# koide3/fast_gicp

Measured on AMD Instinct MI355X. Metric: registrations/sec (100-iter reuse) + final fitness_score; achieved HBM GB/s, higher is better.
Workload: dtype f64

## Files before the change

### fast_gicp_amd/csrc/host_runtime.inc.hpp

```cpp


constexpr int MAX_COST_BLOCKS = MAX_PARTIAL_ROWS;

struct DevBuf {
  void* p = nullptr;
  size_t cap = 0;
  hipError_t ensure(size_t bytes) {
    if (bytes <= cap) return hipSuccess;
    if (p) { hipError_t e = hipFree(p); p = nullptr; cap = 0; if (e != hipSuccess) return e; }
    size_t want = bytes + bytes / 4 + 256;
    hipError_t e = hipMalloc(&p, want);
    if (e == hipSuccess) cap = want;
    return e;
  }
  void release() { if (p) (void)hipFree(p); p = nullptr; cap = 0; }
  template <typename T> T* as() const { return reinterpret_cast<T*>(p); }
};

inline const char* fvh_env(const char* name) { return getenv(name); }
inline long long fvh_env_ll(const char* name, long long dflt) { const char* v = fvh_env(name); return v ? atoll(v) : dflt; }
inline unsigned long long fvh_env_ull(const char* name, unsigned long long dflt) { const char* v = fvh_env(name); return v ? strtoull(v, nullptr, 10) : dflt; }
constexpr int COHERENT_MIN_POINTS = 32768;
struct ProcessParams { int slot_max_split, contended_slot_pct, xcd_local, small_grid_layout; };
inline const ProcessParams& process_params() {
  static const ProcessParams p = [] {
    ProcessParams q;
    q.slot_max_split = (int)std::max(1LL, fvh_env_ll("FVH_SLOT_MAX_SPLIT", 4));
    q.contended_slot_pct = (int)std::min(100LL, std::max(10LL, fvh_env_ll("FVH_CONTENDED_SLOT_PCT", 100)));
    q.xcd_local = fvh_env_ll("FVH_XCD_LOCAL", 1) != 0 ? 1 : 0;
    q.small_grid_layout = fvh_env_ll("FVH_SMALL_GRID_LAYOUT", 2) == 0 ? 0 : 2;
    return q;
  }();
  return p;
}
inline const fvh_engine_params& env_engine_defaults() {
  static const fvh_engine_params d = [] {
    fvh_engine_params p;
    std::memset(&p, 0, sizeof(p));
    p.struct_size = (int)sizeof(fvh_engine_params);
    p.sort_mode = (int)fvh_env_ll("FVH_SORT_MODE", 2);
    p.sort_items = (int)fvh_env_ll("FVH_SORT_ITEMS", 0);
    { const int b = (int)fvh_env_ll("FVH_SORT_FUSED_BITS", 10); p.sort_fused_bits = (b == 9 || b == 10) ? b : 0; }
    p.sort_two_pass_max = (int)fvh_env_ll("FVH_SORT_TWO_PASS_MAX", 262144);
    p.sort_coop_watchdog_ticks = 2'000'000ull;
    p.knn_nearest_first_max_points = (int)fvh_env_ll("FVH_KNN_NEAREST_FIRST_MAX_POINTS", 65536);
    { const int b = (int)fvh_env_ll("FVH_KNN_BLOCK", 64); p.knn_block = (b == 256 || b == 128) ? b : 64; }
    p.coherent_min_points = (int)fvh_env_ll("FVH_COHERENT_MIN_POINTS", COHERENT_MIN_POINTS);
    p.bitmap_min_points = (int)fvh_env_ll("FVH_BITMAP_MIN_POINTS", 300000);
    p.bitmap_max_bytes = std::min(fvh_env_ull("FVH_BITMAP_MAX_BYTES", 32ull << 20), 16ull << 30);
    p.persistent = (int)fvh_env_ll("FVH_PERSISTENT", 1);
    p.persist_watchdog_ticks = 5'000'000ull;
    p.peer_watchdog_ticks = fvh_env_ull("FVH_PEER_WATCHDOG_TICKS", 200'000'000ull);
    p.lm_everywhere = (int)fvh_env_ll("FVH_LM_EVERYWHERE", 1);
    { const char* v = fvh_env("FVH_COST_PRIO"); p.cost_prio = v ? (atoi(v) != 0 ? 1 : 0) : -1; }
    p.cost_split = (int)fvh_env_ll("FVH_COST_SPLIT", 1);
    p.cost_group_max = (int)std::min<long long>(std::max(1LL, fvh_env_ll("FVH_COST_GROUP_MAX", COST_CH)), COST_CH);
    { const long long b = fvh_env_ll("FVH_COST_MAX_BLOCKS", MAX_PARTIAL_ROWS); p.cost_max_blocks = (int)(b < 1 ? 1 : (b > MAX_PARTIAL_ROWS ? MAX_PARTIAL_ROWS : b)); }
    p.cost_target_items = fvh_env_ll("FVH_COST_TARGET_ITEMS", 256LL * 256 * 2);
    p.zerocopy_result = (int)fvh_env_ll("FVH_ZEROCOPY_RESULT", 1);
    { const char* v = fvh_env("FVH_HOST_WAIT"); p.host_wait_block = (v && std::string(v) == "block") ? 1 : 0; }
    p.result_query_spins = fvh_env_ull("FVH_RESULT_QUERY_SPINS", 1024ull);
    p.side_stream = fvh_env_ll("FVH_SIDE_STREAM", 1) != 0 ? 1 : 0;
    p.pinned_upload_max = fvh_env_ull("FVH_PINNED_UPLOAD_MAX", 8ull << 20);
    p.zerocopy_upload_max = fvh_env_ull("FVH_ZEROCOPY_UPLOAD_MAX", 1ull << 20);
    p.avg_fused = fvh_env_ll("FVH_AVG_FUSED", 1) != 0 ? 1 : 0;
    p.nn1_seed = fvh_env_ll("FVH_NN1_SEED", 1) != 0 ? 1 : 0;
    return p;
  }();
  return d;
}
inline const char* check_engine_params(const fvh_engine_params& p) {
  if (p.struct_size != (int)sizeof(fvh_engine_params)) return "engine params: struct_size does not match this library's fvh_engine_params (start from fvh_default_engine_params / fvh_*_get_engine_params)";
  if (p.sort_mode < 0 || p.sort_mode > 3) return "engine params: sort_mode must be 0..3";
  if (p.sort_fused_bits != 0 && p.sort_fused_bits != 9 && p.sort_fused_bits != 10) return "engine params: sort_fused_bits must be 0, 9 or 10";
  if (p.knn_block != 64 && p.knn_block != 128 && p.knn_block != 256) return "engine params: knn_block must be 64, 128 or 256";
  if (p.cost_group_max < 1 || p.cost_group_max > COST_CH) return "engine params: cost_group_max must be 1..4";
  if (p.cost_max_blocks < 1 || p.cost_max_blocks > MAX_PARTIAL_ROWS) return "engine params: cost_max_blocks must be 1..1024";
  if (p.cost_target_items < 1) return "engine params: cost_target_items must be positive";
  if (p.lm_everywhere < 0 || p.lm_everywhere > 2 || p.cost_prio < -1 || p.cost_prio > 1) return "engine params: lm_everywhere must be 0..2, cost_prio -1..1";
  if (p.bitmap_max_bytes > (16ull << 30)) return "engine params: bitmap_max_bytes beyond 16 GiB (the LM kernel indexes its words with 32 bits)";
  if (p.sort_items < 0 || p.sort_items > SORT_ITEMS_MAX || (p.sort_items & 63)) return "engine params: sort_items must be 0 or a multiple of 64 up to 1024";
  return nullptr;
}
// ... 118 lines not shown
  Grant acquire(int dev, int cap, int want) {
    std::lock_guard<std::mutex> lk(mu);
    dev &= 15;
    const auto now = std::chrono::steady_clock::now();
    active[dev]++;
    if (active[dev] > 1) last_contention[dev] = now;
    else if (recent[dev] > 1 && now - last_contention[dev] > std::chrono::milliseconds(QUIET_RESET_MS)) { recent[dev] = 1; calm[dev] = 0; }
    recent[dev] = std::max(recent[dev], active[dev]);
    const int max_split = process_params().slot_max_split;
    const int contended_pct = process_params().contended_slot_pct;
    const bool contended = recent[dev] > 1;
    const int pool = contended ? cap * contended_pct / 100 : cap;
    const int share = std::max(1, pool / std::max(1, std::min(recent[dev], max_split)));
    Grant g;
    g.n = std::min(std::min(want, share), std::max(0, cap - reserved[dev]));
    if (g.n < std::min(want, 32)) {
      active[dev]--;
      calm[dev] = 0;
      last_contention[dev] = now;
      return Grant{};
    }
    reserved[dev] += g.n;
    return g;
  }
  void snapshot(int dev, int* res, int* act, int* rec) {
    std::lock_guard<std::mutex> lk(mu);
    dev &= 15;
    *res = reserved[dev]; *act = active[dev]; *rec = recent[dev];
  }
  void release(int dev, const Grant& g) {
    std::lock_guard<std::mutex> lk(mu);
    dev &= 15;
    reserved[dev] -= g.n;
    active[dev]--;
    if (recent[dev] > active[dev] + 1) {
      if (++calm[dev] >= DECAY_AFTER) { recent[dev]--; calm[dev] = 0; }
    } else {
      calm[dev] = 0;
    }
  }
};
SlotPool g_slots;
constexpr int XCD_LOCAL_MAX_STRIKES = 3;
std::atomic<int> g_xcd_local_strikes{0};
inline bool xcd_local_wanted() {
  return process_params().xcd_local && g_xcd_local_strikes.load() < XCD_LOCAL_MAX_STRIKES;
}
struct GridPlan { int nb = 0; int ng = 0; int local = 0; };
inline int small_grid_layout() {
  return process_params().small_grid_layout;
}
inline int default_groups(int nb) {
  if (nb > SINGLE_LEVEL_MAX_BLOCKS) return TICKET_GROUPS;
  return (small_grid_layout() == 2 && nb >= 2 * TICKET_GROUPS) ? TICKET_GROUPS : 1;
}
```

### fast_gicp_amd/csrc/kernels_cost.hpp

```cpp
#pragma once
#include <cstddef>
#include <type_traits>

#include "dev_math.hpp"
#include "kernels_peer.hpp"
#include "kernels_voxelmap.hpp"

#pragma clang fp contract(on)

namespace fvh {

constexpr int NSUM = 28;
constexpr int PART_STRIDE = 32;
constexpr int MAX_PARTIAL_ROWS = 1024;

enum CostMode { MODE_VGICP = 0, MODE_NDT_P2D = 1, MODE_NDT_D2D = 2 };
enum Phase { PH_LINEARIZE = 0, PH_TRIAL = 1, PH_DONE = 2, PH_FIND_ONLY = 3, PH_EVAL_DERIV = 4, PH_EVAL_ERROR = 5,
             PH_TRIAL_FINAL = 6 };

struct LmState {
  PoseD x0;
  PoseD xi;
  PoseD x_lin;
  double H[36], b[6], d[6];
// ... 140 lines not shown
  if (__builtin_amdgcn_ballot_w64(rot_eps > 0 && trans_eps > 0) != 0ull) {
    bool ok = true;
#pragma unroll
    for (int i = 0; i < 9; i++) ok &= (fabs(delta.r[i] - ((i % 4 == 0) ? 1.0 : 0.0)) < rot_eps);
#pragma unroll
    for (int i = 0; i < 3; i++) ok &= (fabs(delta.t[i]) < trans_eps);
    return ok;
  }
  double rmax = 0, tmax = 0;
#pragma unroll
  for (int i = 0; i < 9; i++) rmax = fmax(rmax, fabs(delta.r[i] - ((i % 4 == 0) ? 1.0 : 0.0)));
#pragma unroll
  for (int i = 0; i < 3; i++) tmax = fmax(tmax, fabs(delta.t[i]));
  const double qr = rmax / rot_eps, qt = tmax / trans_eps;
  return (qr < qt ? qt : qr) < 1;
}

__device__ __host__ inline void unpack_sums(const double* s, double* H, double* b) {
  for (int i = 0; i < 6; i++) b[i] = s[1 + i];
  const double* rr = s + 7;
  const double* rt = s + 13;
  const double* tt = s + 22;
  const int sym[3][3] = {{0, 1, 2}, {1, 3, 4}, {2, 4, 5}};
  for (int i = 0; i < 3; i++)
    for (int j = 0; j < 3; j++) {
      H[i * 6 + j] = rr[sym[i][j]];
      H[i * 6 + 3 + j] = rt[i * 3 + j];
      H[(3 + j) * 6 + i] = rt[i * 3 + j];
      H[(3 + i) * 6 + 3 + j] = tt[sym[i][j]];
    }
}
__device__ __host__ constexpr int sums_index_of_H(int i, int j) {
  const int a = i < 3 ? i : i - 3, c = j < 3 ? j : j - 3;
  const int lo = a < c ? a : c, hi = a < c ? c : a;
  const int sym = lo * 3 - (lo * (lo - 1)) / 2 + (hi - lo);
  return (i < 3 && j < 3) ? 7 + sym : (i >= 3 && j >= 3) ? 22 + sym : (i < 3) ? 13 + i * 3 + (j - 3) : 13 + j * 3 + (i - 3);
}

#ifdef FVH_LM_STEP_NOINLINE
#define FVH_LM_STEP_ATTR __noinline__
#else
#define FVH_LM_STEP_ATTR __forceinline__
#endif
#define FVH_UNI(c) (__builtin_amdgcn_ballot_w64(c) != 0ull)
#ifdef FVH_COST_TIMING
__device__ unsigned long long g_lmtime[16][8];
__device__ unsigned g_lmcall;
#endif
#if defined(FVH_COST_TIMING) && defined(FVH_LM_STAGES)
#define FVH_LM_T(k) do { asm volatile("s_waitcnt vmcnt(0) lgkmcnt(0)" ::: "memory"); if (lane == 0 && lm_call < 16) g_lmtime[lm_call][k] = __builtin_readcyclecounter(); } while (0)
#else
#define FVH_LM_T(k) do { } while (0)
#endif
template <bool GN = false>
__device__ FVH_LM_STEP_ATTR void dev_lm_step_wave(LmState* st, const double* sums, const int lane, double* trace = nullptr) {
  const bool in36 = lane < 36, in12 = lane < 12, in6 = lane < 6;
  double* x0p = reinterpret_cast<double*>(&st->x0);
  double* xip = reinterpret_cast<double*>(&st->xi);
  double* xlp = reinterpret_cast<double*>(&st->x_lin);
#if defined(FVH_COST_TIMING) && defined(FVH_LM_STAGES)
  const unsigned lm_call = __builtin_amdgcn_readfirstlane(g_lmcall);
  if (lane == 0) g_lmcall = lm_call + 1;
#endif
  FVH_LM_T(0);
  const int phase0 = __builtin_amdgcn_readfirstlane(st->phase);
  int phase = phase0;
  double lambda = st->lambda, nu = st->nu, y0 = st->y0;
  int outer_iter = __builtin_amdgcn_readfirstlane(st->outer_iter), inner_iter = __builtin_amdgcn_readfirstlane(st->inner_iter);
  int converged = __builtin_amdgcn_readfirstlane(st->converged), lm_failed = __builtin_amdgcn_readfirstlane(st->lm_failed);
  int num_linearize = __builtin_amdgcn_readfirstlane(st->num_linearize), num_error_evals = __builtin_amdgcn_readfirstlane(st->num_error_evals);
  int nr_iterations = __builtin_amdgcn_readfirstlane(st->nr_iterations), corr_cur = __builtin_amdgcn_readfirstlane(st->corr_cur);
  const int max_iterations = __builtin_amdgcn_readfirstlane(st->max_iterations), lm_max_iterations = __builtin_amdgcn_readfirstlane(st->lm_max_iterations);
  constexpr bool gauss_newton = GN;
  const double rot_eps = st->rotation_epsilon, trans_eps = st->transformation_epsilon, lambda_factor = st->lm_init_lambda_factor;
  double dprev[6], bprev[6];
#pragma unroll
  for (int j = 0; j < 6; j++) { dprev[j] = st->d[j]; bprev[j] = st->b[j]; }
  const int delta_conv_prev = __builtin_amdgcn_readfirstlane(st->delta_converged);

  const double s0 = sums[0], s28 = sums[28];
  if (lane == 0 && sums[30] > 0.0) st->halo_exceeded = 1;

  bool accepted = false, consume = false, done = false;
  if (phase0 == PH_LINEARIZE) {
    consume = true;
  } else {
    const double yi = phase0 == PH_TRIAL_FINAL ? s0 : s28;
    num_error_evals++;
    double denom = 0;
#pragma unroll
    for (int j = 0; j < 6; j++) denom += dprev[j] * (lambda * dprev[j] - bprev[j]);
    double rho;
    if (FVH_UNI(fabs(denom) > 1e-290)) rho = (y0 - yi) * fast_rcp(denom); else rho = (y0 - yi) / denom;
    if (trace) {
      double dn = 0;
#pragma unroll
      for (int j = 0; j < 6; j++) dn += dprev[j] * dprev[j];
      if (lane == 0) {
        double* row = trace + 6 * (size_t)(num_error_evals - 1);
        row[0] = (double)inner_iter; row[1] = y0; row[2] = yi; row[3] = rho; row[4] = lambda; row[5] = sqrt(dn);
      }
    }
    const bool conv = delta_conv_prev != 0;
    if (FVH_UNI(rho < 0)) {
      if (conv) {
        converged = 1; outer_iter++; phase = PH_DONE; done = true;
      } else {
        lambda = nu * lambda;
        nu = 2 * nu;
        inner_iter++;
        if (inner_iter >= lm_max_iterations) { lm_failed = 1; phase = PH_DONE; done = true; }
      }
    } else {
      accepted = true;
      { const double u = 2 * rho - 1; lambda = lambda * fmax(1.0 / 3.0, 1 - u * u * u); }
      converged = conv ? 1 : 0;
      outer_iter++;
      if (converged || outer_iter >= max_iterations) {
        phase = PH_DONE; done = true;
      } else {
        corr_cur ^= 1;
        consume = true;
      }
    }
  }
  FVH_LM_T(1);
  double Hl[21], bv[6];
  if (!done) {
    if (consume) {
      y0 = s0;
#pragma unroll
      for (int i = 0; i < 6; i++) {
        bv[i] = sums[1 + i];
#pragma unroll
        for (int j = 0; j <= i; j++) Hl[i * (i + 1) / 2 + j] = sums[sums_index_of_H(i, j)];
      }
      num_linearize++;
      nr_iterations = outer_iter;
      if (FVH_UNI(lambda < 0.0)) {
        double mx = 0;
#pragma unroll
        for (int i = 0; i < 6; i++) mx = fmax(mx, fabs(Hl[i * (i + 1) / 2 + i]));
        lambda = lambda_factor * mx;
      }
      nu = 2.0;
      inner_iter = 0;
      if (phase0 == PH_LINEARIZE && !gauss_newton) {
        if (lm_max_iterations <= 0) { lm_failed = 1; phase = PH_DONE; done = true; } else phase = PH_TRIAL;
      }
    } else {
#pragma unroll
      for (int i = 0; i < 6; i++) {
        bv[i] = bprev[i];
#pragma unroll
        for (int j = 0; j <= i; j++) Hl[i * (i + 1) / 2 + j] = st->H[i * 6 + j];
      }
    }
  }
  if (lane == 0) { st->lambda = lambda; st->nu = nu; st->y0 = y0; }
  FVH_LM_T(2);
  PoseD delta;
  double d[6];
  bool gn_step = false;
  int delta_conv = delta_conv_prev;
  if (!done) {
    double L[15], D[6], Dinv[6];
    const double lam_solve = gauss_newton ? 0.0 : lambda;
#pragma unroll
    for (int j = 0; j < 6; j++) {
      double dj = Hl[j * (j + 1) / 2 + j] + lam_solve;
#pragma unroll
      for (int k = 0; k < j; k++) dj -= L[j * (j - 1) / 2 + k] * L[j * (j - 1) / 2 + k] * D[k];
      D[j] = dj;
      const double r = fast_rcp(dj);
      const bool pivot_ok = fabs(dj) > 2.2250738585072014e-308;
      Dinv[j] = pivot_ok ? r : 0.0;
      const double scale = pivot_ok ? r : 1.0;
#pragma unroll
      for (int i = j + 1; i < 6; i++) {
        double sacc = Hl[i * (i + 1) / 2 + j];
#pragma unroll
        for (int k = 0; k < j; k++) sacc -= L[i * (i - 1) / 2 + k] * L[j * (j - 1) / 2 + k] * D[k];
        L[i * (i - 1) / 2 + j] = sacc * scale;
      }
    }
    double y[6];
#pragma unroll
    for (int i = 0; i < 6; i++) {
      double sacc = -bv[i];
#pragma unroll
      for (int k = 0; k < i; k++) sacc -= L[i * (i - 1) / 2 + k] * y[k];
      y[i] = sacc;
    }
#pragma unroll
    for (int i = 0; i < 6; i++) y[i] *= Dinv[i];
#pragma unroll
    for (int i = 5; i >= 0; i--) {
      double sacc = y[i];
#pragma unroll
      for (int k = i + 1; k < 6; k++) sacc -= L[k * (k - 1) / 2 + i] * d[k];
      d[i] = sacc;
    }
    FVH_LM_T(3);
    dev_se3_exp(d, delta);
    FVH_LM_T(4);
    delta_conv = FVH_UNI(dev_is_converged(rot_eps, trans_eps, delta)) ? 1 : 0;
    if (gauss_newton) {
      gn_step = true;
      converged = delta_conv;
      outer_iter++;
      phase = (converged || outer_iter >= max_iterations) ? PH_DONE : PH_LINEARIZE;
    } else {
      phase = (delta_conv || outer_iter + 1 >= max_iterations) ? PH_TRIAL_FINAL : PH_TRIAL;
    }
  }
  FVH_LM_T(5);
  double x0r[12], xir[12];
  {
    const double* src = accepted ? xip : x0p;
#pragma unroll
    for (int k = 0; k < 12; k++) x0r[k] = src[k];
  }
  if (accepted && in36) st->final_H[lane] = st->H[lane];
  if (consume) {
    const int li = lane / 6, lj = lane - li * 6;
    const int a = li < 3 ? li : li - 3, c = lj < 3 ? lj : lj - 3;
    const int lo = a < c ? a : c, hi = a < c ? c : a;
    const int sym = lo * 3 - (lo * (lo - 1)) / 2 + (hi - lo);
    int hidx;
    if (li < 3 && lj < 3) hidx = 7 + sym;
    else if (li >= 3 && lj >= 3) hidx = 22 + sym;
    else if (li < 3) hidx = 13 + li * 3 + (lj - 3);
    else hidx = 13 + lj * 3 + (li - 3);
    if (in36) st->H[lane] = sums[hidx];
    if (in6) st->b[lane] = sums[1 + lane];
    if (gn_step && in36) st->final_H[lane] = sums[hidx];
  }
  if (!done) {
#pragma unroll
    for (int i = 0; i < 3; i++) {
#pragma unroll
      for (int j = 0; j < 3; j++) xir[i * 3 + j] = delta.r[i * 3 + 0] * x0r[0 * 3 + j] + delta.r[i * 3 + 1] * x0r[1 * 3 + j] + delta.r[i * 3 + 2] * x0r[2 * 3 + j];
      xir[9 + i] = delta.r[i * 3 + 0] * x0r[9] + delta.r[i * 3 + 1] * x0r[10] + delta.r[i * 3 + 2] * x0r[11] + delta.t[i];
    }
  }
  if (lane == 0) {
    if (accepted) {
#pragma unroll
      for (int k = 0; k < 12; k++) x0p[k] = x0r[k];
    }
    if (consume) {
#pragma unroll
      for (int k = 0; k < 12; k++) xlp[k] = (gn_step && phase != PH_DONE) ? xir[k] : x0r[k];
    }
    if (gn_step) {
#pragma unroll
      for (int k = 0; k < 12; k++) x0p[k] = xir[k];
    }
    if (!done) {
#pragma unroll
      for (int k = 0; k < 12; k++) xip[k] = xir[k];
#pragma unroll
      for (int j = 0; j < 6; j++) st->d[j] = d[j];
    }
    st->phase = phase;
    st->outer_iter = outer_iter; st->inner_iter = inner_iter; st->converged = converged; st->lm_failed = lm_failed;
    st->num_linearize = num_linearize; st->num_error_evals = num_error_evals; st->nr_iterations = nr_iterations; st->corr_cur = corr_cur;
    st->delta_converged = delta_conv;
  }
  FVH_LM_T(6);
}

__global__ void lm_init_kernel(LmState* st, PoseD guess, double rot_eps, double trans_eps, double lambda_factor, int max_iter, int lm_max_iter, unsigned* ticket, int optimizer = 0) {
  if (blockIdx.x == 0 && threadIdx.x <= 8) ticket[threadIdx.x] = 0;
  if (threadIdx.x != 0 || blockIdx.x != 0) return;
  st->x0 = guess; st->xi = guess;
  st->rotation_epsilon = rot_eps; st->transformation_epsilon = trans_eps; st->lm_init_lambda_factor = lambda_factor;
  st->max_iterations = max_iter; st->lm_max_iterations = lm_max_iter; st->optimizer = optimizer; st->pad_ = 0;
  st->lambda = -1.0; st->nu = 2.0; st->y0 = 0.0;
  st->phase = max_iter > 0 ? PH_LINEARIZE : PH_DONE;
  st->corr_cur = 0; st->x_lin = guess; st->delta_converged = 0; st->halo_exceeded = 0;
  st->outer_iter = 0; st->inner_iter = 0; st->converged = 0; st->lm_failed = 0; st->num_linearize = 0; st->num_error_evals = 0; st->nr_iterations = 0;
  for (int i = 0; i < 36; i++) st->final_H[i] = (i % 7 == 0) ? 1.0 : 0.0;
}
template <bool GN = false>
__global__ __launch_bounds__(64) void lm_update_kernel(LmState* st) {
  __shared__ LmState s;
  constexpr int WORDS = sizeof(LmState) / 8 - 1;
  unsigned long long* g = reinterpret_cast<unsigned long long*>(st);
  unsigned long long* l = reinterpret_cast<unsigned long long*>(&s);
  for (int i = threadIdx.x; i < WORDS; i += 64) l[i] = g[i];
  __syncthreads();
  if (s.phase == PH_DONE) return;
  dev_lm_step_wave<GN>(&s, s.sums, threadIdx.x);
  __syncthreads();
  for (int i = threadIdx.x; i < WORDS; i += 64) g[i] = l[i];
}

template <typename Real>
struct ItemAcc {
  Sym3<Real> S;
  Vec3<Real> g;
  Real err;
};
template <typename Real>
__device__ __forceinline__ void hit_term(ItemAcc<Real>& it, const Vec3<Real>& q, const Vec3<Real>& mu, const Sym3<Real>& A, Real w, bool deriv) {
  const Vec3<Real> e = {mu.x - q.x, mu.y - q.y, mu.z - q.z};
  Real det;
  const Sym3<Real> C = adjugate(A, det);
  const Real s = fast_div(w, det);
  const Vec3<Real> Ce = mul(C, e);
  it.err += s * (e.x * Ce.x + e.y * Ce.y + e.z * Ce.z);
  if (!deriv) return;
  it.g.x += s * Ce.x; it.g.y += s * Ce.y; it.g.z += s * Ce.z;
  it.S.xx += s * C.xx; it.S.xy += s * C.xy; it.S.xz += s * C.xz; it.S.yy += s * C.yy; it.S.yz += s * C.yz; it.S.zz += s * C.zz;
}
template <typename Real>
__device__ __forceinline__ Real record_weight(const float4& q3) { return (Real)__hiloint2double(__float_as_int(q3.w), __float_as_int(q3.z)); }
template <typename Real>
__device__ __forceinline__ Real record_weight(const float2&) { return (Real)1; }
template <typename Real>
__device__ __forceinline__ void item_sums(double* v, const ItemAcc<Real>& it, const Vec3<Real>& q) {
  v[0] = (double)it.err;
  const Vec3<Real> bq = cross(it.g, q);
  v[1] = (double)bq.x; v[2] = (double)bq.y; v[3] = (double)bq.z;
  v[4] = -(double)it.g.x; v[5] = -(double)it.g.y; v[6] = -(double)it.g.z;
  const Sym3<Real>& S = it.S;
  const Vec3<Real> c0 = {S.xx, S.xy, S.xz}, c1 = {S.xy, S.yy, S.yz}, c2 = {S.xz, S.yz, S.zz};
  const Vec3<Real> p0 = cross(q, c0), p1 = cross(q, c1), p2 = cross(q, c2);
  const Vec3<Real> r0 = {p0.x, p1.x, p2.x}, r1 = {p0.y, p1.y, p2.y}, r2 = {p0.z, p1.z, p2.z};
  const Vec3<Real> h0 = cross(q, r0), h1 = cross(q, r1), h2 = cross(q, r2);
  v[7] = (double)h0.x; v[8] = (double)h0.y; v[9] = (double)h0.z; v[10] = (double)h1.y; v[11] = (double)h1.z; v[12] = (double)h2.z;
  v[13] = (double)r0.x; v[14] = (double)r0.y; v[15] = (double)r0.z;
  v[16] = (double)r1.x; v[17] = (double)r1.y; v[18] = (double)r1.z;
  v[19] = (double)r2.x; v[20] = (double)r2.y; v[21] = (double)r2.z;
  v[22] = (double)S.xx; v[23] = (double)S.xy; v[24] = (double)S.xz; v[25] = (double)S.yy; v[26] = (double)S.yz; v[27] = (double)S.zz;
}

__device__ __forceinline__ int probe_continue(const unsigned long long* __restrict__ keys, unsigned mask, unsigned long long key, unsigned slot) {
  for (unsigned it = 0; it < mask; it++) {
    slot = (slot + 1) & mask;
    const unsigned long long k = keys[slot];
    if (k == key) return (int)slot;
    if (k == FVH_EMPTY_KEY) return -1;
  }
  return -1;
}
// ... 84 lines not shown
#ifdef FVH_ASM_MARKS
#define FVH_MT(trip, k) asm volatile("; FVH_MARK " #k)
#define FVH_MARK(k) asm volatile("; FVH_MARK " #k)
#else
#define FVH_MT(trip, k) do { } while (0)
#endif
#endif
#ifndef FVH_MARK
#define FVH_MARK(k) do { } while (0)
#endif

#ifndef FVH_COST_WG_PER_CU
#define FVH_COST_WG_PER_CU 3
#endif
#define FVH_COST_BOUNDS __launch_bounds__(256, FVH_COST_WG_PER_CU)
template <typename Real> using LdsPose = const Pose<Real> __attribute__((address_space(3)))*;
typedef const int __attribute__((address_space(3)))* LdsInt;
template <typename Real>
__device__ __forceinline__ Pose<Real> lds_pose(LdsPose<Real> p, int which) {
  Pose<Real> o;
#pragma unroll
  for (int k = 0; k < 9; k++) o.r[k] = p[which].r[k];
#pragma unroll
  for (int k = 0; k < 3; k++) o.t[k] = p[which].t[k];
  return o;
}

constexpr size_t GANG_TICKET_WORDS = 16;
constexpr size_t GANG_BCAST_DOUBLES = (size_t)PERSIST_REPLICAS * BCAST_PAIRS * 2;
constexpr size_t GANG_RESULT_WORDS = (sizeof(LmState) / 8 + 1 + 7) & ~(size_t)7;
constexpr int MAX_GANGS = 64;
struct GangParams {
  int nb_h;
  const PoseD* guesses;
};

template <typename Real, int MODE, bool PERSIST, int CH, bool GN, bool GANG>
__device__ __forceinline__ void cost_body(const CostParams& P, const unsigned gang_lb, const unsigned gang_nb, const unsigned gang, const PoseD* gang_guesses) {
  static_assert(CH == 1 || CH == COST_CH, "one or COST_CH lookups per item");
  auto lin_arg = [&]() -> PoseD { if constexpr (GANG) return gang_guesses[gang]; else return P.lin; };
  auto partials = [&]() -> double* { if constexpr (GANG) return P.partials + (size_t)gang * PARTIALS_DOUBLES; else return P.partials; };
  auto ticket = [&]() -> unsigned* { if constexpr (GANG) return P.ticket + (size_t)gang * GANG_TICKET_WORDS; else return P.ticket; };
  auto bcast_base = [&]() -> double* { if constexpr (GANG) return P.bcast + (size_t)gang * GANG_BCAST_DOUBLES; else return P.bcast; };
  auto corr_base = [&]() -> int* { if constexpr (GANG) return P.corr + (size_t)gang * 2 * P.corr_stride; else return P.corr; };
  auto result_host = [&]() -> unsigned long long* { if constexpr (GANG) return P.result_host ? P.result_host + (size_t)gang * GANG_RESULT_WORDS : nullptr; else return P.result_host; };
#ifdef FVH_COST_TIMING
  __shared__ unsigned long long stamp[12];
  if (threadIdx.x == 0) { stamp[0] = wall_clock64(); atomicMin(&g_cost_timing[0], stamp[0]); }
#endif
  __shared__ double red[4][PART_STRIDE];
  __shared__ double fin[8][PART_STRIDE];
  __shared__ int s_last;
  __shared__ LmState s_st;
  static_assert(sizeof(LmState) % 8 == 0, "LmState is copied as 64-bit words");
  constexpr int ST_WORDS = sizeof(LmState) / 8 - 1;
  static_assert(ST_WORDS <= 256, "one state word per thread after the barrier");
  LmState* st = GANG ? P.st + gang : P.st;
  unsigned long long* st_words = reinterpret_cast<unsigned long long*>(st);
  const unsigned lb = GANG ? gang_lb : blockIdx.x, nb = GANG ? gang_nb : gridDim.x;
  unsigned gen = 0;
  int phase, corr_sel;
  PoseD lin_d, ev_d;
  if (P.host_phase >= 0) {
    phase = P.host_phase;
    lin_d = P.lin;
    ev_d = P.ev;
    corr_sel = P.host_corr_sel;
  } else if (P.init) {
    phase = PH_LINEARIZE;
    lin_d = lin_arg();
    ev_d = lin_arg();
    corr_sel = 0;
  } else {
    phase = st->phase;
    if (phase == PH_DONE) return;
    lin_d = st->x_lin;
    ev_d = (phase == PH_LINEARIZE) ? st->x0 : st->xi;
    corr_sel = st->corr_cur;
  }
  __shared__ Pose<Real> s_pose[2];
  if (threadIdx.x == 0) { s_pose[0] = pose_cast<Real>(lin_d); s_pose[1] = pose_cast<Real>(ev_d); }
  __shared__ int s_grid[8];
  __shared__ int s_region[8];
  constexpr int OFFP_LDS = 64;
  __shared__ int s_offp[OFFP_LDS];
  if (threadIdx.x >= 64 && threadIdx.x < 64 + OFFP_LDS) s_offp[threadIdx.x - 64] = ((int)threadIdx.x - 64 < P.n_off) ? P.offsets_packed[threadIdx.x - 64] : 0;
  if (threadIdx.x < 8) {
    const int t = threadIdx.x;
    int gv = 0, rv = 0;
    if (P.bitmap && P.grid) gv = t < 3 ? P.grid->b0[t] : (t < 6 ? P.grid->nb[t - 3] : (t == 6 ? P.grid->enabled : 0));
    if (P.region) rv = t < 3 ? P.region->inner_lo[t] : (t < 6 ? P.region->inner_hi[t - 3] : 0);
    s_grid[t] = gv; s_region[t] = rv;
  }
  __syncthreads();
  const int n_src_launch = P.d_n_src ? *P.d_n_src : P.n_src;
  constexpr int STICKY_T = PERSIST ? 256 : 1;
  __shared__ float4 s_src[3][STICKY_T];
  constexpr int ELEM_ITS = 2;
  __shared__ int s_elem[PERSIST ? ELEM_ITS : 1][STICKY_T];
  __shared__ int s_ids[2][CH][STICKY_T];
  __shared__ int s_ofp[CH][STICKY_T];
  bool a_primed = false;
  for (;;) {
  if (PERSIST) FVH_PT_MIN(gen, 0);
  const bool fused = (P.host_phase < 0) && (phase == PH_TRIAL);
  constexpr bool EXT_OK = !PERSIST && MODE == MODE_VGICP;
// ... 406 lines not shown
      double s = 0.0;
#pragma unroll
      for (int c = 0; c < 8; c++) s += fin[c][v];
      red[0][v] = s;
    }
  };
  auto init_state = [&]() {
    s_st.x0 = lin_arg(); s_st.xi = lin_arg(); s_st.x_lin = lin_arg();
    s_st.rotation_epsilon = P.rotation_epsilon; s_st.transformation_epsilon = P.transformation_epsilon; s_st.lm_init_lambda_factor = P.lm_init_lambda_factor;
    s_st.max_iterations = P.max_iterations; s_st.lm_max_iterations = P.lm_max_iterations; s_st.optimizer = P.optimizer; s_st.pad_ = 0;
    s_st.lambda = -1.0; s_st.nu = 2.0; s_st.y0 = 0.0;
    s_st.phase = PH_LINEARIZE; s_st.corr_cur = 0; s_st.delta_converged = 0; s_st.halo_exceeded = 0;
    s_st.outer_iter = 0; s_st.inner_iter = 0; s_st.converged = 0; s_st.lm_failed = 0; s_st.num_linearize = 0; s_st.num_error_evals = 0; s_st.nr_iterations = 0;
    for (int i = 0; i < 36; i++) s_st.final_H[i] = (i % 7 == 0) ? 1.0 : 0.0;
  };

  if constexpr (!PERSIST) {
    if (tid == 0) s_last = (atomicAdd(&ticket()[grp], 1u) == gsize - 1);
    __syncthreads();
    if (!s_last) return;
    FVH_STAMP(3);
    reduce_group_rows((size_t)MAX_PARTIAL_ROWS + grp);
    if (tid == 0) s_last = (atomicAdd(&ticket()[TICKET_GROUPS], 1u) == ngroups - 1);
    __syncthreads();
    if (!s_last) return;
    FVH_STAMP(4);

    reduce_final((size_t)MAX_PARTIAL_ROWS);
    if (tid <= TICKET_GROUPS) ticket()[tid] = 0;
    if (MODE == MODE_VGICP && P.peer.n > 1) {
      __syncthreads();
      if (!peer_exchange_sums(P.peer, red[0], P.peer.xbase, P.peer_watchdog_ticks, tid, 256, &s_last)) {
        if (tid == 0) __hip_atomic_store(&st->aborted, 2u, __ATOMIC_RELAXED, __HIP_MEMORY_SCOPE_AGENT);
        return;
      }
    }
    for (int i = tid; i < ST_WORDS; i += 256) reinterpret_cast<unsigned long long*>(&s_st)[i] = st_words[i];
    int vm_nv = 0, vm_dr = 0, vm_nv2 = 0;
    if (tid == 0) {
      vm_nv = P.vm_counters[0];
      vm_nv2 = P.vm_counters2 ? P.vm_counters2[0] : 0;
      vm_dr = P.vm_counters[1] + (P.vm_counters2 ? P.vm_counters2[1] : 0);
    }
    __syncthreads();
    FVH_STAMP(5);
    if (tid == 0) {
      for (int v = 0; v < PART_STRIDE; v++) s_st.sums[v] = red[0][v];
      s_st.vm_num_voxels = vm_nv;
      s_st.vm_num_voxels2 = vm_nv2;
      s_st.vm_dropped = vm_dr;
      if (P.host_phase < 0 && P.init) init_state();
    }
    __syncthreads();
    if (P.host_phase < 0 && !P.defer_lm && tid < 64) dev_lm_step_wave<GN>(&s_st, red[0], tid, P.lm_trace);
    FVH_STAMP(6);
    __syncthreads();
    for (int i = tid; i < ST_WORDS; i += 256) st_words[i] = reinterpret_cast<const unsigned long long*>(&s_st)[i];
#ifdef FVH_COST_TIMING
    asm volatile("s_waitcnt vmcnt(0)" ::: "memory");
    if (tid == 0) {
      stamp[7] = wall_clock64();
      for (int i = 1; i <= 7; i++) g_cost_timing[i] = stamp[i];
      g_cost_timing[8] = nb;
      g_cost_timing[9] = stamp[0];
    }
#endif
    return;
  } else {
    const unsigned trip = gen;
    unsigned long long ltag = P.launch_tag;
    asm volatile("" : "+s"(ltag));
    auto want_tag_of = [&]() { unsigned long long t = ltag * 4096ull + trip + 1; asm volatile("" : "+s"(t)); return (double)t; };
    auto abort_tag_of = [&]() { unsigned long long t = ltag * 4096ull; asm volatile("" : "+s"(t)); return -(double)t; };
    __shared__ double bc[BCAST_PAIRS];
    __shared__ unsigned s_abort;
    pair_t* wrows = reinterpret_cast<pair_t*>(partials() + WG_ROWS_OFFSET);
    pair_t* trows = reinterpret_cast<pair_t*>(partials() + TAGGED_ROWS_OFFSET) + (size_t)(trip & 1u) * (TICKET_GROUPS + 1) * PART_STRIDE;
    pair_t* bcast = reinterpret_cast<pair_t*>(bcast_base());
    const bool local = P.xcd_local != 0;
    const unsigned reps = NG == 1 ? (unsigned)PERSIST_REPLICAS : (unsigned)(PERSIST_REPLICAS / TICKET_GROUPS);
    static_assert(PERSIST_REPLICAS % (2 * TICKET_GROUPS) == 0, "an even number of broadcast copies per group");
    pair_t* my_bcast = bcast + (size_t)(NG == 1 ? 0u : grp * reps) * BCAST_PAIRS;
    auto poison = [&](int first, int stride) {
      pair_t pv;
      pv.x = 0.0; pv.y = abort_tag_of();
      for (int idx = first; idx < PERSIST_REPLICAS * BCAST_PAIRS; idx += stride) store_pair_agent(bcast + idx, pv);
    };
    const double my_rot = local ? (double)((__builtin_amdgcn_readfirstlane(xcc_id()) - blockIdx.x) & 7u) : 0.0;
    if (tid < PART_STRIDE) {
      pair_t pv;
      pv.x = (red[0][tid] + red[1][tid]) + (red[2][tid] + red[3][tid]);
      if (tid == PART_STRIDE - 1) pv.x = my_rot;
      pv.y = want_tag_of();
      if (local) store_pair_xcd(wrows + (size_t)lb * PART_STRIDE + tid, pv); else store_pair_agent(wrows + (size_t)lb * PART_STRIDE + tid, pv);
    }
    FVH_PT_MAX(trip, 2);
    const bool collector = lb < NG;
    const bool multi_gpu = MODE == MODE_VGICP && P.peer.n > 1;
    const bool everywhere = P.lm_everywhere != 0 && !multi_gpu;
    const bool adds_rows = collector;
    if (collector || everywhere) {
      if (tid == 0) { s_last = 1; s_abort = 0u; }
      __syncthreads();
      if (adds_rows) {
        const int v = tid & 31, chunk = tid >> 5;
        const double want = want_tag_of();
        double s = 0.0;
        for (unsigned j0 = chunk; j0 < gsize; j0 += 8 * 8) {
          const pair_t* src[8];
          double t[8];
          unsigned pend = 0;
#pragma unroll
          for (int u = 0; u < 8; u++) {
            const unsigned j = j0 + 8 * u;
            const bool in = j < gsize;
            src[u] = wrows + (size_t)(grp + (in ? j : j0) * NG) * PART_STRIDE + v;
            t[u] = 0.0;
            pend |= in ? (1u << u) : 0u;
          }
          const unsigned long long t0 = wall_clock64();
          for (;;) {
            pair_t pv[8];
            load_pairs8_agent(pv, src);
#pragma unroll
            for (int u = 0; u < 8; u++)
              if (((pend >> u) & 1u) && pv[u].y == want) { t[u] = pv[u].x; pend &= ~(1u << u); }
            if (!pend) break;
            if (wall_clock64() - t0 > P.watchdog_ticks) { s_last = 0; break; }
            __builtin_amdgcn_s_sleep(1);
          }
          if (v == PART_STRIDE - 1) {
#pragma unroll
            for (int u = 0; u < 8; u++) t[u] = (((j0 + 8 * u) < gsize) && t[u] != my_rot) ? 1.0 : 0.0;
          }
#pragma unroll
          for (int u = 0; u < 8; u++) s += t[u];
        }
        fin[chunk][v] = s;
      }
      if (adds_rows) __syncthreads();
      if (!s_last) {
        poison(tid, 256);
        if (tid == 0) __hip_atomic_store(&st->aborted, 1u, __ATOMIC_RELAXED, __HIP_MEMORY_SCOPE_AGENT);
        return;
      }
      if (adds_rows && tid < PART_STRIDE) {
        double s = 0.0;
#pragma unroll
        for (int c = 0; c < 8; c++) s += fin[c][tid];
        if (tid == PART_STRIDE - 1) s = (s == 0.0) ? my_rot : -1.0;
        if (NG > 1) {
          pair_t pv;
          pv.x = s; pv.y = want_tag_of();
          store_pair_agent(trows + (size_t)grp * PART_STRIDE + tid, pv);
        }
        red[1][tid] = s;
      }
      FVH_PT_MAX(trip, 5);
      if (tid < 64) {
        const int lane = tid;
        double val = 0.0;
        bool ok = true;
        if (NG == 1) {
          if (lane < PART_STRIDE) val = red[1][lane];
        } else if (!multi_gpu || lb == 0) {
          const pair_t* src[8];
          double t[8];
          unsigned pend = 0;
#pragma unroll
          for (int g = 0; g < 8; g++) {
            const bool in = (unsigned)g < NG;
            src[g] = trows + (size_t)(in ? g : 0) * PART_STRIDE + (lane & 31);
            t[g] = 0.0;
            pend |= in ? (1u << g) : 0u;
          }
          if (lane >= PART_STRIDE) pend = 0;
          const double want = want_tag_of();
          const unsigned long long t0 = wall_clock64();
          while (__builtin_amdgcn_ballot_w64(pend != 0u) != 0ull) {
            pair_t pv[8];
            load_pairs8_agent(pv, src);
#pragma unroll
            for (int g = 0; g < 8; g++)
              if (((pend >> g) & 1u) && pv[g].y == want) { t[g] = pv[g].x; pend &= ~(1u << g); }
            if (__builtin_amdgcn_readfirstlane((int)(wall_clock64() - t0 > P.watchdog_ticks))) { ok = false; break; }
          }
          if (lane == PART_STRIDE - 1) {
#pragma unroll
            for (int g = 0; g < 8; g++) t[g] = ((unsigned)g < NG && t[g] != my_rot) ? 1.0 : 0.0;
          }
#pragma unroll
          for (int g = 0; g < 8; g++) val += t[g];
        } else {
          const pair_t* src = trows + (size_t)GLOBAL_ROW * PART_STRIDE + (lane & 31);
          const double want = want_tag_of();
          const unsigned long long t0 = wall_clock64();
          bool pend = lane < PART_STRIDE;
          while (__builtin_amdgcn_ballot_w64(pend) != 0ull) {
            const pair_t pv = load_pair_agent(src);
            if (pend && pv.y == want) { val = pv.x; pend = false; }
            if (__builtin_amdgcn_readfirstlane((int)(wall_clock64() - t0 > P.watchdog_ticks))) { ok = false; break; }
          }
        }
        FVH_PT_MAX(trip, 6);
        if (lane == PART_STRIDE - 1) {
          const bool placement_ok = !local || (NG == 1 ? val == my_rot : val == 0.0);
          if (ok && !placement_ok) s_abort = 3u;
          val = 0.0;
        }
        if (lane < PART_STRIDE) red[0][lane] = val;
        if (!ok && lane == 0) s_abort = 1u;
      }
      if (multi_gpu && lb == 0) {
        __syncthreads();
        if constexpr (MODE == MODE_VGICP) {
          if (!s_abort && !peer_exchange_sums(P.peer, red[0], P.peer.xbase + trip, P.peer_watchdog_ticks, tid, 256, &s_last)) {
            if (tid == 0) s_abort = 2u;
          }
        }
        __syncthreads();
        if (!s_abort && NG > 1 && tid < PART_STRIDE) {
          pair_t pv;
          pv.x = red[0][tid]; pv.y = want_tag_of();
          store_pair_agent(trows + (size_t)GLOBAL_ROW * PART_STRIDE + tid, pv);
        }
      }
      if (tid < 64) {
        const int lane = tid;
        if (__builtin_amdgcn_ballot_w64(s_abort != 0u) == 0ull) {
          FVH_PT_MAX(trip, 7);
          if (trip == 0 && lane == 0) {
            init_state();
            s_st.vm_num_voxels = P.vm_counters[0];
            s_st.vm_num_voxels2 = P.vm_counters2 ? P.vm_counters2[0] : 0;
            s_st.vm_dropped = P.vm_counters[1] + (P.vm_counters2 ? P.vm_counters2[1] : 0);
          }
          if (lane < PART_STRIDE) s_st.sums[lane] = red[0][lane];
          FVH_PT_MAX(trip, 8);
          FVH_MARK(20);
#ifdef FVH_COST_TIMING
          const unsigned long long lm_c0 = __builtin_readcyclecounter();
#endif
          dev_lm_step_wave<GN>(&s_st, red[0], lane, lb == 0 ? P.lm_trace : nullptr);
#ifdef FVH_COST_TIMING
          if (threadIdx.x == 0 && trip < 16 && lb == 0) g_ptime[trip][0][11] = __builtin_readcyclecounter() - lm_c0;
#endif
          FVH_MARK(21);
          FVH_PT_MAX(trip, 9);
          const int ph = __builtin_amdgcn_readfirstlane(s_st.phase);
          double v = 0.0;
          const int d = lane & 31;
          if (d < BCAST_VALUES) {
            const double* xl = reinterpret_cast<const double*>(&s_st.x_lin);
            const double* pe = reinterpret_cast<const double*>(ph == PH_LINEARIZE ? &s_st.x0 : &s_st.xi);
            if (d == 0) v = (double)ph;
            else if (d == 1) v = (double)s_st.corr_cur;
            else if (d < 14) v = xl[d - 2];
            else v = pe[d - 14];
            if (lane < 32) bc[d] = v;
            pair_t pv;
            pv.x = v; pv.y = want_tag_of();
            pair_t* dst = my_bcast + lane;
            static_assert(BCAST_PAIRS == 32, "two copies per store instruction");
            if (everywhere) {
            } else if (local) {
              for (unsigned r = 0; r < reps; r += 2) store_pair_xcd(dst + (size_t)r * BCAST_PAIRS, pv);
            } else {
              for (unsigned r = 0; r < reps; r += 2) store_pair_agent(dst + (size_t)r * BCAST_PAIRS, pv);
            }
          }
          FVH_PT_MAX(trip, 3);
        }
      }
      __syncthreads();
      if (s_abort) {
        poison(tid, 256);
        if (tid == 0) __hip_atomic_store(&st->aborted, s_abort, __ATOMIC_RELAXED, __HIP_MEMORY_SCOPE_AGENT);
        return;
      }
      if (lb == 0 && s_st.phase == PH_DONE) {
        for (int i = tid; i < ST_WORDS; i += 256) st_words[i] = reinterpret_cast<const unsigned long long*>(&s_st)[i];
        if (result_host()) {
          for (int i = tid; i < ST_WORDS; i += 256)
            __hip_atomic_store(&result_host()[i], reinterpret_cast<const unsigned long long*>(&s_st)[i], __ATOMIC_RELAXED, __HIP_MEMORY_SCOPE_SYSTEM);
          asm volatile("s_waitcnt vmcnt(0)" ::: "memory");
          __syncthreads();
          if (tid == 0) __hip_atomic_store(&result_host()[ST_WORDS + 1], P.launch_tag, __ATOMIC_RELEASE, __HIP_MEMORY_SCOPE_SYSTEM);
        }
      }
    } else {
      if (tid < 64) {
        const pair_t* rep = my_bcast + (size_t)((lb / NG) % reps) * BCAST_PAIRS;
        const int lane = tid;
        const bool is_val = lane < BCAST_VALUES;
        const unsigned long long t0 = wall_clock64();
        const double want_tag = want_tag_of(), abort_tag = abort_tag_of();
        int ok = 0;
        for (;;) {
          pair_t pv;
          pv.x = 0.0; pv.y = want_tag;
          if (is_val) pv = load_pair_agent(rep + lane);
          if (__any(is_val && pv.y == abort_tag)) break;
          if (__all(pv.y == want_tag)) {
            if (is_val) bc[lane] = pv.x;
            ok = 1;
            break;
          }
          if (__builtin_amdgcn_readfirstlane((int)(wall_clock64() - t0 > P.watchdog_ticks))) {
            poison(lane, 64);
            if (lane == 0) __hip_atomic_store(&st->aborted, 1u, __ATOMIC_RELAXED, __HIP_MEMORY_SCOPE_AGENT);
            break;
          }
          __builtin_amdgcn_s_sleep(1);
        }
        if (lane == 0) s_last = ok;
      }
      __syncthreads();
      if (!s_last) return;
    }
    FVH_PT_MAX(trip, 4);
    gen++;
    phase = (int)uniform_f64(bc[0]);
    if (phase == PH_DONE) return;
    corr_sel = (int)uniform_f64(bc[1]);
    if (tid < 24) {
      const int which = tid / 12, k = tid % 12;
      const Real v = (Real)bc[2 + tid];
      if (k < 9) s_pose[which].r[k] = v; else s_pose[which].t[k - 9] = v;
    }
    __syncthreads();
  }
  }
}

template <typename Real, int MODE, bool PERSIST, int CH = COST_CH, bool GN = false>
__global__ FVH_COST_BOUNDS void cost_kernel(CostParams P) {
  cost_body<Real, MODE, PERSIST, CH, GN, false>(P, 0u, 0u, 0u, nullptr);
}

template <typename Real, int MODE, bool PERSIST, int CH = COST_CH, bool GN = false>
__global__ FVH_COST_BOUNDS void lm_gang_kernel(CostParams P, GangParams G) {
  const unsigned nb_h = (unsigned)G.nb_h;
  const unsigned gang = blockIdx.x / nb_h;
  cost_body<Real, MODE, PERSIST, CH, GN, true>(P, blockIdx.x - gang * nb_h, nb_h, gang, G.guesses);
}

}
```

Baseline: 5398.

## Split LM step into prefix and rest, overlap prefix with grid reduction

The Levenberg-Marquardt step is split into a prefix (denominator, reciprocal and Hessian index table) and a remainder. The prefix now runs in the persistent cost kernel before the cross-block reduction wait, so it is off the serialized critical path between trips. Tail loads are hoisted, and broadcast pose values are written straight into shared pose registers, which removes a barrier per trip. A new env knob sets the block threshold for grouped ticket layout. This adds shared scratch and changes the ordering of state init against the reduction, which risks subtle races.

```diff
diff --git a/fast_gicp_amd/csrc/host_runtime.inc.hpp b/fast_gicp_amd/csrc/host_runtime.inc.hpp
--- a/fast_gicp_amd/csrc/host_runtime.inc.hpp
+++ b/fast_gicp_amd/csrc/host_runtime.inc.hpp
@@ -21,7 +21,7 @@
 inline long long fvh_env_ll(const char* name, long long dflt) { const char* v = fvh_env(name); return v ? atoll(v) : dflt; }
 inline unsigned long long fvh_env_ull(const char* name, unsigned long long dflt) { const char* v = fvh_env(name); return v ? strtoull(v, nullptr, 10) : dflt; }
 constexpr int COHERENT_MIN_POINTS = 32768;
-struct ProcessParams { int slot_max_split, contended_slot_pct, xcd_local, small_grid_layout; };
+struct ProcessParams { int slot_max_split, contended_slot_pct, xcd_local, small_grid_layout, grouped_min_blocks; };
 inline const ProcessParams& process_params() {
   static const ProcessParams p = [] {
     ProcessParams q;
@@ -29,6 +29,7 @@
     q.contended_slot_pct = (int)std::min(100LL, std::max(10LL, fvh_env_ll("FVH_CONTENDED_SLOT_PCT", 100)));
     q.xcd_local = fvh_env_ll("FVH_XCD_LOCAL", 1) != 0 ? 1 : 0;
     q.small_grid_layout = fvh_env_ll("FVH_SMALL_GRID_LAYOUT", 2) == 0 ? 0 : 2;
+    q.grouped_min_blocks = (int)std::max<long long>(TICKET_GROUPS, fvh_env_ll("FVH_GROUPED_MIN_BLOCKS", 2 * TICKET_GROUPS));
     return q;
   }();
   return p;
@@ -253,5 +254,5 @@
 }
 inline int default_groups(int nb) {
   if (nb > SINGLE_LEVEL_MAX_BLOCKS) return TICKET_GROUPS;
-  return (small_grid_layout() == 2 && nb >= 2 * TICKET_GROUPS) ? TICKET_GROUPS : 1;
-}
+  return (small_grid_layout() == 2 && nb >= process_params().grouped_min_blocks) ? TICKET_GROUPS : 1;
+}
diff --git a/fast_gicp_amd/csrc/kernels_cost.hpp b/fast_gicp_amd/csrc/kernels_cost.hpp
--- a/fast_gicp_amd/csrc/kernels_cost.hpp
+++ b/fast_gicp_amd/csrc/kernels_cost.hpp
@@ -216,9 +216,36 @@
 #else
 #define FVH_LM_T(k) do { } while (0)
 #endif
+struct LmStepScratch {
+  double denom, rden;
+  int hidx[64];
+};
+__device__ __forceinline__ void dev_lm_step_prefix(const LmState* st, LmStepScratch* sc, const int lane) {
+  if (__builtin_amdgcn_readfirstlane(st->phase) != PH_LINEARIZE) {
+    const double lambda = st->lambda;
+    double dprev[6], bprev[6];
+#pragma unroll
+    for (int j = 0; j < 6; j++) { dprev[j] = st->d[j]; bprev[j] = st->b[j]; }
+    double denom = 0;
+#pragma unroll
+    for (int j = 0; j < 6; j++) denom += dprev[j] * (lambda * dprev[j] - bprev[j]);
+    const double rden = fast_rcp(denom);
+    if (lane == 0) { sc->denom = denom; sc->rden = rden; }
+  }
+  const int li = lane / 6, lj = lane - li * 6;
+  const int a = li < 3 ? li : li - 3, c = lj < 3 ? lj : lj - 3;
+  const int lo = a < c ? a : c, hi = a < c ? c : a;
+  const int sym = lo * 3 - (lo * (lo - 1)) / 2 + (hi - lo);
+  int hidx;
+  if (li < 3 && lj < 3) hidx = 7 + sym;
+  else if (li >= 3 && lj >= 3) hidx = 22 + sym;
+  else if (li < 3) hidx = 13 + li * 3 + (lj - 3);
+  else hidx = 13 + lj * 3 + (li - 3);
+  sc->hidx[lane] = lane < 36 ? hidx : 0;
+}
 template <bool GN = false>
-__device__ FVH_LM_STEP_ATTR void dev_lm_step_wave(LmState* st, const double* sums, const int lane, double* trace = nullptr) {
-  const bool in36 = lane < 36, in12 = lane < 12, in6 = lane < 6;
+__device__ FVH_LM_STEP_ATTR void dev_lm_step_rest(LmState* st, const double* sums, const int lane, const LmStepScratch* sc, double* trace = nullptr) {
+  const bool in36 = lane < 36, in6 = lane < 6;
   double* x0p = reinterpret_cast<double*>(&st->x0);
   double* xip = reinterpret_cast<double*>(&st->xi);
   double* xlp = reinterpret_cast<double*>(&st->x_lin);
@@ -237,10 +264,8 @@
   const int max_iterations = __builtin_amdgcn_readfirstlane(st->max_iterations), lm_max_iterations = __builtin_amdgcn_readfirstlane(st->lm_max_iterations);
   constexpr bool gauss_newton = GN;
   const double rot_eps = st->rotation_epsilon, trans_eps = st->transformation_epsilon, lambda_factor = st->lm_init_lambda_factor;
-  double dprev[6], bprev[6];
-#pragma unroll
-  for (int j = 0; j < 6; j++) { dprev[j] = st->d[j]; bprev[j] = st->b[j]; }
   const int delta_conv_prev = __builtin_amdgcn_readfirstlane(st->delta_converged);
+  const double pre_denom = sc->denom, pre_rden = sc->rden;
 
   const double s0 = sums[0], s28 = sums[28];
   if (lane == 0 && sums[30] > 0.0) st->halo_exceeded = 1;
@@ -251,15 +276,13 @@
   } else {
     const double yi = phase0 == PH_TRIAL_FINAL ? s0 : s28;
     num_error_evals++;
-    double denom = 0;
-#pragma unroll
-    for (int j = 0; j < 6; j++) denom += dprev[j] * (lambda * dprev[j] - bprev[j]);
+    const double denom = pre_denom;
     double rho;
-    if (FVH_UNI(fabs(denom) > 1e-290)) rho = (y0 - yi) * fast_rcp(denom); else rho = (y0 - yi) / denom;
+    if (FVH_UNI(fabs(denom) > 1e-290)) rho = (y0 - yi) * pre_rden; else rho = (y0 - yi) / denom;
     if (trace) {
       double dn = 0;
 #pragma unroll
-      for (int j = 0; j < 6; j++) dn += dprev[j] * dprev[j];
+      for (int j = 0; j < 6; j++) dn += st->d[j] * st->d[j];
       if (lane == 0) {
         double* row = trace + 6 * (size_t)(num_error_evals - 1);
         row[0] = (double)inner_iter; row[1] = y0; row[2] = yi; row[3] = rho; row[4] = lambda; row[5] = sqrt(dn);
@@ -315,7 +338,7 @@
     } else {
 #pragma unroll
       for (int i = 0; i < 6; i++) {
-        bv[i] = bprev[i];
+        bv[i] = st->b[i];
 #pragma unroll
         for (int j = 0; j <= i; j++) Hl[i * (i + 1) / 2 + j] = st->H[i * 6 + j];
       }
@@ -327,6 +350,18 @@
   double d[6];
   bool gn_step = false;
   int delta_conv = delta_conv_prev;
+  double x0r[12], xir[12];
+  double hold = 0.0, hnew = 0.0, bnew = 0.0;
+  auto tail_loads = [&]() {
+    const double* src = accepted ? xip : x0p;
+#pragma unroll
+    for (int k = 0; k < 12; k++) x0r[k] = src[k];
+    if (accepted && in36) hold = st->H[lane];
+    if (consume) {
+      if (in36) hnew = sums[sc->hidx[lane]];
+      if (in6) bnew = sums[1 + lane];
+    }
+  };
   if (!done) {
     double L[15], D[6], Dinv[6];
     const double lam_solve = gauss_newton ? 0.0 : lambda;
@@ -379,26 +414,12 @@
     }
   }
   FVH_LM_T(5);
-  double x0r[12], xir[12];
-  {
-    const double* src = accepted ? xip : x0p;
-#pragma unroll
-    for (int k = 0; k < 12; k++) x0r[k] = src[k];
-  }
-  if (accepted && in36) st->final_H[lane] = st->H[lane];
+  tail_loads();
+  if (accepted && in36) st->final_H[lane] = hold;
   if (consume) {
-    const int li = lane / 6, lj = lane - li * 6;
-    const int a = li < 3 ? li : li - 3, c = lj < 3 ? lj : lj - 3;
-    const int lo = a < c ? a : c, hi = a < c ? c : a;
-    const int sym = lo * 3 - (lo * (lo - 1)) / 2 + (hi - lo);
-    int hidx;
-    if (li < 3 && lj < 3) hidx = 7 + sym;
-    else if (li >= 3 && lj >= 3) hidx = 22 + sym;
-    else if (li < 3) hidx = 13 + li * 3 + (lj - 3);
-    else hidx = 13 + lj * 3 + (li - 3);
-    if (in36) st->H[lane] = sums[hidx];
-    if (in6) st->b[lane] = sums[1 + lane];
-    if (gn_step && in36) st->final_H[lane] = sums[hidx];
+    if (in36) st->H[lane] = hnew;
+    if (in6) st->b[lane] = bnew;
+    if (gn_step && in36) st->final_H[lane] = hnew;
   }
   if (!done) {
 #pragma unroll
@@ -433,6 +454,11 @@
     st->delta_converged = delta_conv;
   }
   FVH_LM_T(6);
+}
+template <bool GN = false>
+__device__ __forceinline__ void dev_lm_step_wave(LmState* st, LmStepScratch* sc, const double* sums, const int lane, double* trace = nullptr) {
+  dev_lm_step_prefix(st, sc, lane);
+  dev_lm_step_rest<GN>(st, sums, lane, sc, trace);
 }
 
 __global__ void lm_init_kernel(LmState* st, PoseD guess, double rot_eps, double trans_eps, double lambda_factor, int max_iter, int lm_max_iter, unsigned* ticket, int optimizer = 0) {
@@ -450,13 +476,14 @@
 template <bool GN = false>
 __global__ __launch_bounds__(64) void lm_update_kernel(LmState* st) {
   __shared__ LmState s;
+  __shared__ LmStepScratch s_sc;
   constexpr int WORDS = sizeof(LmState) / 8 - 1;
   unsigned long long* g = reinterpret_cast<unsigned long long*>(st);
   unsigned long long* l = reinterpret_cast<unsigned long long*>(&s);
   for (int i = threadIdx.x; i < WORDS; i += 64) l[i] = g[i];
   __syncthreads();
   if (s.phase == PH_DONE) return;
-  dev_lm_step_wave<GN>(&s, s.sums, threadIdx.x);
+  dev_lm_step_wave<GN>(&s, &s_sc, s.sums, threadIdx.x);
   __syncthreads();
   for (int i = threadIdx.x; i < WORDS; i += 64) g[i] = l[i];
 }
@@ -647,6 +674,7 @@
   __shared__ double fin[8][PART_STRIDE];
   __shared__ int s_last;
   __shared__ LmState s_st;
+  __shared__ LmStepScratch s_lmsc;
   static_assert(sizeof(LmState) % 8 == 0, "LmState is copied as 64-bit words");
   constexpr int ST_WORDS = sizeof(LmState) / 8 - 1;
   static_assert(ST_WORDS <= 256, "one state word per thread after the barrier");
@@ -1159,7 +1187,7 @@
       if (P.host_phase < 0 && P.init) init_state();
     }
     __syncthreads();
-    if (P.host_phase < 0 && !P.defer_lm && tid < 64) dev_lm_step_wave<GN>(&s_st, red[0], tid, P.lm_trace);
+    if (P.host_phase < 0 && !P.defer_lm && tid < 64) dev_lm_step_wave<GN>(&s_st, &s_lmsc, red[0], tid, P.lm_trace);
     FVH_STAMP(6);
     __syncthreads();
     for (int i = tid; i < ST_WORDS; i += 256) st_words[i] = reinterpret_cast<const unsigned long long*>(&s_st)[i];
@@ -1180,6 +1208,12 @@
     auto want_tag_of = [&]() { unsigned long long t = ltag * 4096ull + trip + 1; asm volatile("" : "+s"(t)); return (double)t; };
     auto abort_tag_of = [&]() { unsigned long long t = ltag * 4096ull; asm volatile("" : "+s"(t)); return -(double)t; };
     __shared__ double bc[BCAST_PAIRS];
+    auto put_payload = [&](const int d, const double v) {
+      if (d < 2) { bc[d] = v; return; }
+      const int which = (d - 2) / 12, k = (d - 2) % 12;
+      const Real vr = (Real)v;
+      if (k < 9) s_pose[which].r[k] = vr; else s_pose[which].t[k - 9] = vr;
+    };
     __shared__ unsigned s_abort;
     pair_t* wrows = reinterpret_cast<pair_t*>(partials() + WG_ROWS_OFFSET);
     pair_t* trows = reinterpret_cast<pair_t*>(partials() + TAGGED_ROWS_OFFSET) + (size_t)(trip & 1u) * (TICKET_GROUPS + 1) * PART_STRIDE;
@@ -1264,10 +1298,17 @@
         red[1][tid] = s;
       }
       FVH_PT_MAX(trip, 5);
+      double val = 0.0;
       if (tid < 64) {
         const int lane = tid;
-        double val = 0.0;
         bool ok = true;
+        if (trip == 0 && lane == 0) {
+          init_state();
+          s_st.vm_num_voxels = P.vm_counters[0];
+          s_st.vm_num_voxels2 = P.vm_counters2 ? P.vm_counters2[0] : 0;
+          s_st.vm_dropped = P.vm_counters[1] + (P.vm_counters2 ? P.vm_counters2[1] : 0);
+        }
+        dev_lm_step_prefix(&s_st, &s_lmsc, lane);
         if (NG == 1) {
           if (lane < PART_STRIDE) val = red[1][lane];
         } else if (!multi_gpu || lb == 0) {
@@ -1336,19 +1377,14 @@
         const int lane = tid;
         if (__builtin_amdgcn_ballot_w64(s_abort != 0u) == 0ull) {
           FVH_PT_MAX(trip, 7);
-          if (trip == 0 && lane == 0) {
-            init_state();
-            s_st.vm_num_voxels = P.vm_counters[0];
-            s_st.vm_num_voxels2 = P.vm_counters2 ? P.vm_counters2[0] : 0;
-            s_st.vm_dropped = P.vm_counters[1] + (P.vm_counters2 ? P.vm_counters2[1] : 0);
-          }
-          if (lane < PART_STRIDE) s_st.sums[lane] = red[0][lane];
+          if (multi_gpu && lb == 0 && lane < PART_STRIDE) val = red[0][lane];
+          if (lane < PART_STRIDE) s_st.sums[lane] = val;
           FVH_PT_MAX(trip, 8);
           FVH_MARK(20);
 #ifdef FVH_COST_TIMING
           const unsigned long long lm_c0 = __builtin_readcyclecounter();
 #endif
-          dev_lm_step_wave<GN>(&s_st, red[0], lane, lb == 0 ? P.lm_trace : nullptr);
+          dev_lm_step_rest<GN>(&s_st, red[0], lane, &s_lmsc, lb == 0 ? P.lm_trace : nullptr);
 #ifdef FVH_COST_TIMING
           if (threadIdx.x == 0 && trip < 16 && lb == 0) g_ptime[trip][0][11] = __builtin_readcyclecounter() - lm_c0;
 #endif
@@ -1364,7 +1400,7 @@
             else if (d == 1) v = (double)s_st.corr_cur;
             else if (d < 14) v = xl[d - 2];
             else v = pe[d - 14];
-            if (lane < 32) bc[d] = v;
+            if (lane < 32) put_payload(d, v);
             pair_t pv;
             pv.x = v; pv.y = want_tag_of();
             pair_t* dst = my_bcast + lane;
@@ -1409,7 +1445,7 @@
           if (is_val) pv = load_pair_agent(rep + lane);
           if (__any(is_val && pv.y == abort_tag)) break;
           if (__all(pv.y == want_tag)) {
-            if (is_val) bc[lane] = pv.x;
+            if (is_val) put_payload(lane, pv.x);
             ok = 1;
             break;
           }
@@ -1430,12 +1466,6 @@
     phase = (int)uniform_f64(bc[0]);
     if (phase == PH_DONE) return;
     corr_sel = (int)uniform_f64(bc[1]);
-    if (tid < 24) {
-      const int which = tid / 12, k = tid % 12;
-      const Real v = (Real)bc[2 + tid];
-      if (k < 9) s_pose[which].r[k] = v; else s_pose[which].t[k - 9] = v;
-    }
-    __syncthreads();
   }
   }
 }
```

New measurement: 5436 (median of 3 runs). No clear change (+0.7%).
